# techpro-studio/NNToolkitCore

Hardware: AMD Instinct MI355X
Metric: audio frames/sec (whole node) (higher is better)
Workload: dtype f32

## Files before the change

### nntoolkitcore_amd/csrc/hip/conv1d_kernels.hpp

```cpp
#pragma once
#include "nntk_common.hpp"
#include <stdlib.h>
#include <type_traits>

#define CONV_BM 128
#define CONV_KC 16
#define CONV_LS (CONV_KC + 4)

struct ConvParams {
    const float *in;
    long in_seq, in_row;
    const float *wp;
    const float *bias;
    const float *bn;
    float *out;
    float bn_eps;
    float relu_a;
    int act_kind;
    int B, T, Cin, Cin_p, Cout, Cout_p, k, stride, Tout;
    int tiles_per_seq;
    int m_tiles, n_tiles;
    int out_mode;
    int rows_a;
    int bn_fast;
// ... 276 lines not shown
    if (fast_store) {
        if (!p.bn && p.act_kind == NNTK_ACT_IDENTITY) epilogue(F_{}, AId{}, T_{});
        else if (p.bn && p.act_kind == NNTK_ACT_RELU) epilogue(T_{}, ARelu{}, T_{});
        else if (p.bn)                                epilogue(T_{}, AAny{}, T_{});
        else                                          epilogue(F_{}, AAny{}, T_{});
    } else {
        if (p.bn) epilogue(T_{}, AAny{}, F_{});
        else      epilogue(F_{}, AAny{}, F_{});
    }
}

typedef __bf16 cf3_bf16x2 __attribute__((ext_vector_type(2)));
typedef float cf3_f32x2 __attribute__((ext_vector_type(2)));
__device__ __forceinline__ unsigned cf3_cvt_pk(float a, float b) {
    return __builtin_bit_cast(unsigned, __builtin_convertvector((cf3_f32x2){a, b}, cf3_bf16x2));
}
__device__ __forceinline__ void cf3_split_pair(float x0, float x1, unsigned &hi, unsigned &mid, unsigned &lo) {
#pragma clang fp contract(off)
    hi = cf3_cvt_pk(x0, x1);
    const float r0 = x0 - __uint_as_float(hi << 16), r1 = x1 - __uint_as_float(hi & 0xffff0000u);
    mid = cf3_cvt_pk(r0, r1);
    const float s0 = r0 - __uint_as_float(mid << 16), s1 = r1 - __uint_as_float(mid & 0xffff0000u);
    lo = cf3_cvt_pk(s0, s1);
}

#define CONV_F3_BB 8
#define CONV_F3_TT 16
#ifndef CONV_F3_TMAJOR
#define CONV_F3_BL(m) ((m) & 7)
#define CONV_F3_TL(m) ((m) >> 3)
#else
#define CONV_F3_BL(m) ((m) >> 4)
#define CONV_F3_TL(m) ((m) & 15)
#endif

template <int TM, int TN, int WN>
__device__ __forceinline__ void conv_epilogue_frag3(const ConvParams &p, f32x16 (&acc)[TM][TN], int b0, int x0, int n0,
                                                    int wm, int wn, int l31, int kh, const float *cst) {
    constexpr int BN = WN * TN * 32;
    const size_t total = (size_t)p.Tout * p.f3_nht * p.f3_nks * 3 * 1024;
    const __amdgpu_buffer_rsrc_t rs_out = conv_rsrc(p.out, total);
    auto epilogue = [&](auto bn_tag, auto act_tag) {
        constexpr bool HAS_BN = decltype(bn_tag)::value;
        constexpr int ACT = decltype(act_tag)::value;
        int row_voff[TM];
#pragma unroll
        for (int i = 0; i < TM; ++i) {
            const int m = (wm * TM + i) * 32 + l31;
            const int b = b0 + CONV_F3_BL(m), x = x0 + CONV_F3_TL(m);
            row_voff[i] = (b < p.B && x < p.Tout) ? (int)((((size_t)x * p.f3_nht + (b >> 5)) * p.f3_nks * 3) * 1024) + (32 * kh + (b & 31)) * 16
                                                  : CONV_OOB;
        }
#pragma unroll
        for (int j = 0; j < TN; ++j) {
#pragma unroll
            for (int gp = 0; gp < 2; ++gp) {
                const int cu = n0 + (wn * TN + j) * 32 + 16 * gp;
                const bool ks_ok = cu < p.Cout;
                const int ks_off = (cu >> 4) * 3 * 1024;
                unsigned img[TM][2][3][2];
#pragma unroll
                for (int s = 0; s < 2; ++s) {
                    const int g = 2 * gp + s;
                    const int cb = cu + 8 * s + 4 * kh;
                    const int cl = (wn * TN + j) * 32 + 8 * g + 4 * kh;
                    const float4 bias4 = *reinterpret_cast<const float4 *>(cst + cl);
                    const float bias[4] = {bias4.x, bias4.y, bias4.z, bias4.w};
                    float ga[4] = {1.f, 1.f, 1.f, 1.f}, be[4] = {0.f, 0.f, 0.f, 0.f}, mu[4] = {0.f, 0.f, 0.f, 0.f},
                          sd[4] = {1.f, 1.f, 1.f, 1.f}, rsd[4] = {1.f, 1.f, 1.f, 1.f};
                    if (HAS_BN) {
                        const float4 t1 = *reinterpret_cast<const float4 *>(cst + BN + cl);
                        const float4 t2 = *reinterpret_cast<const float4 *>(cst + 2 * BN + cl);
                        const float4 t3 = *reinterpret_cast<const float4 *>(cst + 3 * BN + cl);
                        const float4 t4 = *reinterpret_cast<const float4 *>(cst + 4 * BN + cl);
                        const float4 t5 = *reinterpret_cast<const float4 *>(cst + 5 * BN + cl);
                        ga[0] = t1.x; ga[1] = t1.y; ga[2] = t1.z; ga[3] = t1.w;
                        be[0] = t2.x; be[1] = t2.y; be[2] = t2.z; be[3] = t2.w;
                        mu[0] = t3.x; mu[1] = t3.y; mu[2] = t3.z; mu[3] = t3.w;
                        sd[0] = t4.x; sd[1] = t4.y; sd[2] = t4.z; sd[3] = t4.w;
                        rsd[0] = t5.x; rsd[1] = t5.y; rsd[2] = t5.z; rsd[3] = t5.w;
                    }
#pragma unroll
                    for (int i = 0; i < TM; ++i) {
                        float v[4];
#pragma unroll
                        for (int e = 0; e < 4; ++e) {
                            v[e] = acc[i][j][4 * g + e] + bias[e];
                            if (HAS_BN) {
                                const float d = v[e] - mu[e];
                                float qn = d * rsd[e];
                                qn = fmaf(fmaf(-qn, sd[e], d), rsd[e], qn);
                                v[e] = p.bn_fast ? (d * rsd[e]) * ga[e] + be[e] : nofma_muladd(qn, ga[e], be[e]);
                            }
                            v[e] = ACT == -1 ? nntk_act(p.act_kind, v[e], p.relu_a)
                                 : ACT == NNTK_ACT_RELU ? nntk_act(NNTK_ACT_RELU, v[e], p.relu_a)
                                 : v[e];
                            if (cb + e >= p.Cout) v[e] = 0.0f;
                        }
                        cf3_split_pair(v[0], v[1], img[i][s][0][0], img[i][s][1][0], img[i][s][2][0]);
                        cf3_split_pair(v[2], v[3], img[i][s][0][1], img[i][s][1][1], img[i][s][2][1]);
                    }
                }
#pragma unroll
                for (int i = 0; i < TM; ++i) {
#pragma unroll
                    for (int im = 0; im < 3; ++im) {
                        const auto s01 = __builtin_amdgcn_permlane32_swap(img[i][0][im][0], img[i][1][im][0], false, false);
                        const auto s23 = __builtin_amdgcn_permlane32_swap(img[i][0][im][1], img[i][1][im][1], false, false);
                        const v4u32_t pk = {s01[0], s23[0], s01[1], s23[1]};
                        const int vo = (ks_ok && row_voff[i] != CONV_OOB) ? row_voff[i] + ks_off + im * 1024 : CONV_OOB;
                        __builtin_amdgcn_raw_buffer_store_b128(pk, rs_out, vo, 0, 0);
                    }
                }
            }
        }
    };
    using T_ = std::true_type; using F_ = std::false_type;
    using AId = std::integral_constant<int, NNTK_ACT_IDENTITY>;
    using ARelu = std::integral_constant<int, NNTK_ACT_RELU>;
    using AAny = std::integral_constant<int, -1>;
    if (!p.bn && p.act_kind == NNTK_ACT_IDENTITY) epilogue(F_{}, AId{});
    else if (p.bn && p.act_kind == NNTK_ACT_RELU) epilogue(T_{}, ARelu{});
    else if (p.bn)                                epilogue(T_{}, AAny{});
    else                                          epilogue(F_{}, AAny{});
}

template <int WM, int WN, int TM, int TN, bool A4, bool QUAD, int AMAX = 192>
__global__ __launch_bounds__(256, 2) void conv1d_mfma_kernel(ConvParams p) {
    constexpr int BN = WN * TN * 32;
    constexpr int KC = CONV_KC, LS = CONV_LS;
    static_assert(WM * WN == 4, "4 wavefronts per workgroup");
    static_assert(WM * TM * 32 == CONV_BM, "BM = 128");
    extern __shared__ __attribute__((aligned(16))) float smem[];
    const int a_elems = p.rows_a * LS;
    constexpr int w_elems = BN * LS;
    const int w_base = 2 * a_elems;

    const int tid = threadIdx.x;
    const int lane = tid & 63;
    const int wave = __builtin_amdgcn_readfirstlane(tid >> 6);
    const int wm = wave / WN, wn = wave % WN;
    const int l31 = lane & 31, kh = lane >> 5;

    const int xcd = blockIdx.x & 7, local = blockIdx.x >> 3;
    const int tile = (local / p.n_tiles) * 8 + xcd;
    if (tile >= p.m_tiles) return;
    const int b = tile / p.tiles_per_seq;
    const int x0 = (tile % p.tiles_per_seq) * CONV_BM;
    const int n0 = (local % p.n_tiles) * BN;
    const int Ktot = p.k * p.Cin_p;


    f32x16 acc[TM][TN];

    constexpr int A_TPR = A4 ? KC / 4 : KC;
    constexpr int AR_STEP = 256 / A_TPR;
    constexpr int A_PT = (AMAX + AR_STEP - 1) / AR_STEP;
    constexpr int W_PT = (BN * (KC / 4) + 255) / 256;
    constexpr bool W_ALL = (BN * (KC / 4)) % 256 == 0;
    const int ac = A4 ? (tid % A_TPR) * 4 : (tid % A_TPR);
    const int ar = tid / A_TPR;
    const int wr = tid >> 2, wc4 = tid & 3;
    v4u32_t areg4[A4 ? A_PT : 1];
    unsigned areg[A4 ? 1 : A_PT];
    v4u32_t wreg[W_PT];
    int a_voff[A_PT], w_voff[W_PT];
#pragma unroll
    for (int q = 0; q < A_PT; ++q) a_voff[q] = (int)(((long)(ar + q * AR_STEP) * p.in_row + ac) * 4);
#pragma unroll
    for (int q = 0; q < W_PT; ++q) w_voff[q] = ((wr + q * 64) * Ktot + wc4 * 4) * 4;
    const bool cin_ragged = (p.Cin % KC) != 0;

    const int n_cchunks = p.Cin_p / KC;
    const int n_chunks = n_cchunks * p.k;
    const int last_blocks = (((p.Cin + 7) & ~7) - (n_cchunks - 1) * KC + 7) / 8;

    const __amdgpu_buffer_rsrc_t rs_w = conv_rsrc(p.wp, (size_t)p.Cout_p * Ktot * 4);
    auto load_w = [&](int tn0, int cc, int kk) {
        const int soff = (tn0 * Ktot + kk * p.Cin_p + cc * KC) * 4;
#pragma unroll
        for (int q = 0; q < W_PT; ++q)
            if (W_ALL || tid + q * 256 < BN * (KC / 4))
                wreg[q] = __builtin_amdgcn_raw_buffer_load_b128(rs_w, w_voff[q], soff, 0);
    };
    const size_t in_total = (size_t)p.B * p.T * p.Cin;
    auto load_a = [&](int tb, int tx0, int cc) {
        const size_t in_off = (size_t)tb * p.in_seq + (size_t)tx0 * p.stride * p.in_row;
        const __amdgpu_buffer_rsrc_t rs_in = conv_rsrc(p.in + in_off, (in_total - in_off) * 4);
        const int soff = cc * KC * 4;
        if (cin_ragged && cc == n_cchunks - 1) {
            const bool ch_ok = cc * KC + ac < p.Cin;
#pragma unroll
            for (int q = 0; q < A_PT; ++q) {
                const int vo = ch_ok ? a_voff[q] : CONV_OOB;
                if (A4) areg4[q] = __builtin_amdgcn_raw_buffer_load_b128(rs_in, vo, soff, 0);
                else    areg[q] = __builtin_amdgcn_raw_buffer_load_b32(rs_in, vo, soff, 0);
            }
        } else {
#pragma unroll
            for (int q = 0; q < A_PT; ++q) {
                if (A4) areg4[q] = __builtin_amdgcn_raw_buffer_load_b128(rs_in, a_voff[q], soff, 0);
                else    areg[q] = __builtin_amdgcn_raw_buffer_load_b32(rs_in, a_voff[q], soff, 0);
            }
        }
    };

    const int a_rd = ((wm * TM * 32 + l31) * p.stride) * LS + 4 * kh;
    const int w_rd = w_base + (wn * TN * 32 + l31) * LS + 4 * kh;
    const int a_tile = 32 * p.stride * LS;

    load_a(b, x0, 0);
    load_w(n0, 0, 0);
    float *cst = smem + 2 * a_elems + 2 * w_elems;
    {
        float c[6];
        conv_load_constants<BN>(p, n0, tid, c);
        conv_stage_constants<BN>(cst, tid, c);
    }
#pragma unroll
    for (int i = 0; i < TM; ++i)
#pragma unroll
        for (int j = 0; j < TN; ++j)
#pragma unroll
            for (int r = 0; r < 16; ++r) acc[i][j][r] = 0.0f;
    int cc = 0, kk = 0;
    for (int chunk = 0; chunk < n_chunks; ++chunk) {
        const int wbuf = chunk & 1;
        const int abuf = cc & 1;
        if (kk == 0) {
            float *As = smem + abuf * a_elems;
#pragma unroll
            for (int q = 0; q < A_PT; ++q) {
                const int r = ar + q * AR_STEP;
                if (r < p.rows_a) {
                    if (A4) *reinterpret_cast<v4u32_t *>(As + r * LS + ac) =
                                (cin_ragged && cc == n_cchunks - 1) ? mask_channels(areg4[q], p.Cin - (cc * KC + ac)) : areg4[q];
                    else    *reinterpret_cast<unsigned *>(As + r * LS + ac) = areg[q];
                }
            }
        }
        {
            float *Ws = smem + w_base + wbuf * w_elems;
#pragma unroll
            for (int q = 0; q < W_PT; ++q)
                if (W_ALL || tid + q * 256 < BN * (KC / 4))
                    *reinterpret_cast<v4u32_t *>(Ws + (wr + q * 64) * LS + wc4 * 4) = wreg[q];
        }
        __syncthreads();
        int ncc = cc, nkk = kk + 1;
        if (nkk == p.k) { nkk = 0; ncc = cc + 1; }
        if (chunk + 1 < n_chunks && !CONV_DBG(4)) {
            load_w(n0, ncc, nkk);
            if (nkk == 0) load_a(b, x0, ncc);
        }
        const float *A = smem + abuf * a_elems + kk * LS + a_rd;
        const float *W = smem + wbuf * w_elems + w_rd;
        auto block8 = [&](int s) {
            float4 a[TM], w[TN];
#pragma unroll
            for (int i = 0; i < TM; ++i) a[i] = *reinterpret_cast<const float4 *>(A + i * a_tile + s);
#pragma unroll
            for (int j = 0; j < TN; ++j) w[j] = *reinterpret_cast<const float4 *>(W + j * 32 * LS + s);
#pragma unroll
            for (int u = 0; u < 4; ++u)
#pragma unroll
                for (int i = 0; i < TM; ++i)
#pragma unroll
                    for (int j = 0; j < TN; ++j) {
                        const float av = u == 0 ? a[i].x : u == 1 ? a[i].y : u == 2 ? a[i].z : a[i].w;
                        const float wv = u == 0 ? w[j].x : u == 1 ? w[j].y : u == 2 ? w[j].z : w[j].w;
                        acc[i][j] = QUAD ? __builtin_amdgcn_mfma_f32_32x32x2f32(wv, av, acc[i][j], 0, 0, 0)
                                         : __builtin_amdgcn_mfma_f32_32x32x2f32(av, wv, acc[i][j], 0, 0, 0);
                    }
        };
        if (!CONV_DBG(2)) {
        block8(0);
        if (cc != n_cchunks - 1 || last_blocks > 1) block8(8);
        }
        cc = ncc; kk = nkk;
    }

    if (CONV_DBG(1) && acc[0][0][0] != 12345.678f) return;
    if constexpr (QUAD) conv_epilogue<TM, TN, WN>(p, acc, b, x0, n0, wm, wn, l31, kh, cst);
    else conv_epilogue_rows<TM, TN, WN>(p, acc, b, x0, n0, wm, wn, l31, kh, cst);
}

typedef __bf16 bf16x8_t __attribute__((ext_vector_type(8)));
typedef __bf16 bf16x2_t __attribute__((ext_vector_type(2)));
typedef float f32x2_t __attribute__((ext_vector_type(2)));

__device__ __forceinline__ unsigned cvt_pk_bf16(float a, float b) {
    return __builtin_bit_cast(unsigned, __builtin_convertvector((f32x2_t){a, b}, bf16x2_t));
}
__device__ __forceinline__ void split3_pair(float x0, float x1, unsigned &hi, unsigned &mid, unsigned &lo) {
    hi = cvt_pk_bf16(x0, x1);
    const float r0 = x0 - __uint_as_float(hi << 16), r1 = x1 - __uint_as_float(hi & 0xffff0000u);
    mid = cvt_pk_bf16(r0, r1);
    const float s0 = r0 - __uint_as_float(mid << 16), s1 = r1 - __uint_as_float(mid & 0xffff0000u);
    lo = cvt_pk_bf16(s0, s1);
}

#define SPLIT_ROW 96

template <int WM, int WN, int TM, int TN, bool A4, bool QUAD, int AMAX = 192, bool F3OUT = false>
__global__ __launch_bounds__(256, 2) void conv1d_mfma_bf16x3_kernel(ConvParams p) {
    constexpr int BN = WN * TN * 32;
    constexpr int KC = CONV_KC;
    static_assert(WM * WN == 4 && WM * TM * 32 == CONV_BM, "4 wavefronts, BM = 128");
    static_assert(!F3OUT || QUAD, "the frag3 epilogue is written for the quad orientation");
    extern __shared__ __attribute__((aligned(16))) float smem[];
    char *lds = reinterpret_cast<char *>(smem);
    const int a_bytes = p.rows_a * SPLIT_ROW;
    constexpr int w_bytes = (BN / 32) * 3 * 1024;
    const int w_base = 2 * a_bytes;

    const int tid = threadIdx.x;
    const int lane = tid & 63;
    const int wave = __builtin_amdgcn_readfirstlane(tid >> 6);
    const int wm = wave / WN, wn = wave % WN;
    const int l31 = lane & 31, kh = lane >> 5;

    const int xcd = blockIdx.x & 7, local = blockIdx.x >> 3;
#ifndef CONV_F3_INTERLEAVED
    const int tile = F3OUT ? xcd * ((p.m_tiles + 7) >> 3) + local / p.n_tiles : (local / p.n_tiles) * 8 + xcd;
#else
    const int tile = (local / p.n_tiles) * 8 + xcd;
#endif
    if (tile >= p.m_tiles) return;
    const int b = F3OUT ? (tile / p.tiles_per_seq) * CONV_F3_BB : tile / p.tiles_per_seq;
    const int x0 = (tile % p.tiles_per_seq) * (F3OUT ? CONV_F3_TT : CONV_BM);
    const int n0 = (local % p.n_tiles) * BN;
    const int Ktot = p.k * p.Cin_p;
    const int ksteps = Ktot >> 4, cin_steps = p.Cin_p >> 4;
    const int wrows = CONV_F3_TT + p.k - 1;

    f32x16 acc[TM][TN];

    constexpr int A_TPR = A4 ? KC / 4 : KC;
    constexpr int AR_STEP = 256 / A_TPR;
    constexpr int A_PT = (AMAX + AR_STEP - 1) / AR_STEP;
    const int ac = A4 ? (tid % A_TPR) * 4 : (tid % A_TPR);
    const int ar = tid / A_TPR;
    v4u32_t areg4[A4 ? A_PT : 1];
    unsigned areg[A4 ? 1 : A_PT];
    constexpr int W_CT = (BN / 32 + 3) / 4;
    v4u32_t wreg[W_CT][3];
    int a_voff[A_PT];
#pragma unroll
    for (int q = 0; q < A_PT; ++q) {
        const int r = ar + q * AR_STEP;
        if (F3OUT) {
            const int bl = r / wrows, tr = r - bl * wrows;
            a_voff[q] = (r < p.rows_a && b + bl < p.B) ? (int)(((long)bl * p.in_seq + (long)tr * p.in_row + ac) * 4) : CONV_OOB;
        } else {
            a_voff[q] = (int)(((long)r * p.in_row + ac) * 4);
        }
    }
    const bool cin_ragged = (p.Cin % KC) != 0;
    const int n_cchunks = p.Cin_p / KC;
    const int n_chunks = n_cchunks * p.k;

    const size_t w_elems_total = (size_t)p.Cout_p * Ktot;
    const int img_bytes = (int)(w_elems_total * 2);
    const __amdgpu_buffer_rsrc_t rs_w = conv_rsrc(p.wp + w_elems_total, (size_t)3 * img_bytes);
    const bool w_thread = wave < BN / 32;
    int w_voff[W_CT];
#pragma unroll
    for (int c = 0; c < W_CT; ++c)
        w_voff[c] = wave + 4 * c < BN / 32 ? (((n0 >> 5) + wave + 4 * c) * ksteps) * 1024 + lane * 16 : CONV_OOB;
    auto load_w = [&](int cc, int kk) {
        const int soff = (kk * cin_steps + cc) * 1024;
#pragma unroll
        for (int c = 0; c < W_CT; ++c)
#pragma unroll
            for (int m = 0; m < 3; ++m) wreg[c][m] = __builtin_amdgcn_raw_buffer_load_b128(rs_w, w_voff[c], soff + m * img_bytes, 0);
    };
    const size_t in_total = (size_t)p.B * p.T * p.Cin;
    const size_t in_off = (size_t)b * p.in_seq + (size_t)x0 * p.stride * p.in_row;
    const __amdgpu_buffer_rsrc_t rs_in = conv_rsrc(p.in + in_off, (in_total - in_off) * 4);
    auto load_a = [&](int cc) {
        const bool ch_ok = !(cin_ragged && cc == n_cchunks - 1) || cc * KC + ac < p.Cin;
#pragma unroll
        for (int q = 0; q < A_PT; ++q) {
            const int vo = ch_ok ? a_voff[q] : CONV_OOB;
            if (A4) areg4[q] = __builtin_amdgcn_raw_buffer_load_b128(rs_in, vo, cc * KC * 4, 0);
            else    areg[q] = __builtin_amdgcn_raw_buffer_load_b32(rs_in, vo, cc * KC * 4, 0);
        }
    };
    auto stage_a = [&](char *As, int nvalid) {
#pragma unroll
        for (int q = 0; q < A_PT; q += (A4 ? 1 : 2)) {
            const int r = ar + q * AR_STEP;
            if (A4) {
                if (r < p.rows_a) {
                    const v4u32_t x = nvalid < 4 ? mask_channels(areg4[q], nvalid) : areg4[q];
                    unsigned h0, m0, l0, h1, m1, l1;
                    split3_pair(__uint_as_float(x.x), __uint_as_float(x.y), h0, m0, l0);
                    split3_pair(__uint_as_float(x.z), __uint_as_float(x.w), h1, m1, l1);
                    char *dst = As + r * SPLIT_ROW + 16 * ((ac >> 3) ^ ((r >> 3) & 1)) + (ac & 7) * 2;
                    *reinterpret_cast<uint2 *>(dst) = make_uint2(h0, h1);
                    *reinterpret_cast<uint2 *>(dst + 32) = make_uint2(m0, m1);
                    *reinterpret_cast<uint2 *>(dst + 64) = make_uint2(l0, l1);
                }
            } else {
                unsigned h, m, l;
                split3_pair(__uint_as_float(areg[q]), __uint_as_float(areg[q + 1 < A_PT ? q + 1 : q]), h, m, l);
#pragma unroll
                for (int e = 0; e < 2; ++e) {
                    const int re = r + e * AR_STEP;
                    if (q + e < A_PT && re < p.rows_a) {
                        char *dst = As + re * SPLIT_ROW + 16 * ((ac >> 3) ^ ((re >> 3) & 1)) + (ac & 7) * 2;
                        *reinterpret_cast<unsigned short *>(dst) = (unsigned short)(e ? h >> 16 : h);
                        *reinterpret_cast<unsigned short *>(dst + 32) = (unsigned short)(e ? m >> 16 : m);
                        *reinterpret_cast<unsigned short *>(dst + 64) = (unsigned short)(e ? l >> 16 : l);
                    }
                }
            }
        }
    };

    const int a_row0 = (wm * TM * 32 + l31) * p.stride;
    int a_row_f3[TM];
#pragma unroll
    for (int i = 0; i < TM; ++i) {
        const int m = (wm * TM + i) * 32 + l31;
        a_row_f3[i] = CONV_F3_BL(m) * wrows + CONV_F3_TL(m);
    }
    const int w_rd = w_base + (wn * TN * 3) * 1024 + lane * 16;
    const int w_wr = w_base + (wave * 3) * 1024 + lane * 16;

    load_a(0);
    load_w(0, 0);
    float *cst = reinterpret_cast<float *>(lds + 2 * a_bytes + 2 * w_bytes);
    {
        float c[6];
        conv_load_constants<BN>(p, n0, tid, c);
        conv_stage_constants<BN>(cst, tid, c);
    }
#pragma unroll
    for (int i = 0; i < TM; ++i)
#pragma unroll
        for (int j = 0; j < TN; ++j)
#pragma unroll
            for (int r = 0; r < 16; ++r) acc[i][j][r] = 0.0f;
    int cc = 0, kk = 0;
    for (int chunk = 0; chunk < n_chunks; ++chunk) {
        const int wbuf = chunk & 1;
        const int abuf = cc & 1;
        if (kk == 0 && !CONV_DBG(16)) stage_a(lds + abuf * a_bytes, (cin_ragged && cc == n_cchunks - 1) ? p.Cin - (cc * KC + ac) : 4);
        if (w_thread) {
#pragma unroll
            for (int c = 0; c < W_CT; ++c) {
                char *dst = lds + wbuf * w_bytes + w_wr + c * 4 * 3 * 1024;
#pragma unroll
                for (int m = 0; m < 3; ++m) *reinterpret_cast<v4u32_t *>(dst + 1024 * m) = wreg[c][m];
            }
        }
        __syncthreads();
        int ncc = cc, nkk = kk + 1;
        if (nkk == p.k) { nkk = 0; ncc = cc + 1; }
        if (chunk + 1 < n_chunks) {
            if (!CONV_DBG(4)) load_w(ncc, nkk);
            if (nkk == 0 && !CONV_DBG(32)) load_a(ncc);
        }
        const char *Ab = lds + abuf * a_bytes;
        const char *Wb = lds + wbuf * w_bytes + w_rd;
        bf16x8_t a[3][TM], w[3][TN];
#pragma unroll
        for (int i = 0; i < TM; ++i) {
            const int row = F3OUT ? a_row_f3[i] + kk : a_row0 + i * 32 * p.stride + kk;
            const char *src = Ab + row * SPLIT_ROW + 16 * (kh ^ ((row >> 3) & 1));
#pragma unroll
            for (int m = 0; m < 3; ++m)
                if (!CONV_DBG(8)) a[m][i] = *reinterpret_cast<const bf16x8_t *>(src + 32 * m);
                else a[m][i] = __builtin_bit_cast(bf16x8_t, wreg[0][m]);
        }
#pragma unroll
        for (int j = 0; j < TN; ++j)
#pragma unroll
            for (int m = 0; m < 3; ++m)
                if (!CONV_DBG(8)) w[m][j] = *reinterpret_cast<const bf16x8_t *>(Wb + (j * 3 + m) * 1024);
                else w[m][j] = __builtin_bit_cast(bf16x8_t, wreg[0][m]);
        constexpr int PA[6] = {2, 0, 1, 1, 0, 0};
        constexpr int PW[6] = {0, 2, 1, 0, 1, 0};
        if (!CONV_DBG(2)) {
#pragma unroll
            for (int t = 0; t < 6; ++t)
#pragma unroll
                for (int i = 0; i < TM; ++i)
#pragma unroll
                    for (int j = 0; j < TN; ++j)
                        acc[i][j] = QUAD ? __builtin_amdgcn_mfma_f32_32x32x16_bf16(w[PW[t]][j], a[PA[t]][i], acc[i][j], 0, 0, 0)
                                         : __builtin_amdgcn_mfma_f32_32x32x16_bf16(a[PA[t]][i], w[PW[t]][j], acc[i][j], 0, 0, 0);
        } else {
#pragma unroll
            for (int i = 0; i < TM; ++i)
#pragma unroll
                for (int j = 0; j < TN; ++j)
#pragma unroll
                    for (int m = 0; m < 3; ++m)
                        acc[i][j][m] += __builtin_bit_cast(v4u32_t, a[m][i]).x + __builtin_bit_cast(v4u32_t, w[m][j]).x;
        }
        cc = ncc; kk = nkk;
    }
    if (CONV_DBG(1) && acc[0][0][0] != 12345.678f) return;
    if constexpr (F3OUT) conv_epilogue_frag3<TM, TN, WN>(p, acc, b, x0, n0, wm, wn, l31, kh, cst);
    else if constexpr (QUAD) {
        v4u32_t *epi = nullptr;
#ifndef CONV_EPI_DIRECT
        if (2 * a_bytes + 2 * w_bytes >= CONV_EPI_LDS_BYTES && p.out_mode == 0) {
            __syncthreads();
            epi = reinterpret_cast<v4u32_t *>(lds);
        }
#endif
        conv_epilogue<TM, TN, WN>(p, acc, b, x0, n0, wm, wn, l31, kh, cst, epi);
    }
    else conv_epilogue_rows<TM, TN, WN>(p, acc, b, x0, n0, wm, wn, l31, kh, cst);
}

template <int WM, int WN, int TM, int TN, bool A4>
static int launch_mfma_f3(const ConvParams &p) {
    constexpr int BN = WN * TN * 32;
    size_t lds = (size_t)2 * (p.rows_a * SPLIT_ROW + (BN / 32) * 3 * 1024) + 6 * BN * sizeof(float);
    ConvParams q = p;
    q.m_tiles = ((p.B + CONV_F3_BB - 1) / CONV_F3_BB) * p.tiles_per_seq;
    q.n_tiles = p.Cout_p / BN;
    const long blocks = (long)((q.m_tiles + 7) / 8) * 8 * q.n_tiles;
    if ((long)((p.B + CONV_F3_BB - 1) / CONV_F3_BB) * p.tiles_per_seq > 0x7fffffffL / 8 || blocks > 0x7fffffffL)
        return nntk_fail_msg("conv1d: too many tiles for one launch");
    auto kern = conv1d_mfma_bf16x3_kernel<WM, WN, TM, TN, A4, true, 192, true>;
    if (lds > 64 * 1024) {
        if (nntk_set_max_dynamic_lds((const void *)kern, lds)) return -1;
    }
    hipLaunchKernelGGL(kern, dim3((unsigned)blocks), dim3(256), lds, nntk_stream(), q);
    NNTK_LAUNCH_CHECK("conv1d_mfma_bf16x3_kernel<frag3>");
    nntk_set_last_conv_kernel("conv1d_mfma_bf16x3_kernel<frag3>");
    return 0;
}

template <int WM, int WN, int TM, int TN, bool A4, bool SPLIT, bool QUAD, int AMAX = 192>
static int launch_mfma_o(const ConvParams &p) {
    constexpr int BN = WN * TN * 32;
    size_t lds = SPLIT ? (size_t)2 * (p.rows_a * SPLIT_ROW + (BN / 32) * 3 * 1024)
                       : (size_t)(2 * p.rows_a * CONV_LS + 2 * BN * CONV_LS) * sizeof(float);
    lds += 6 * BN * sizeof(float);
    ConvParams q = p;
    q.m_tiles = p.B * p.tiles_per_seq;
    q.n_tiles = p.Cout_p / BN;
    const long blocks = (long)((q.m_tiles + 7) / 8) * 8 * q.n_tiles;
    if ((long)p.B * p.tiles_per_seq > 0x7fffffffL / 8 || blocks > 0x7fffffffL)
        return nntk_fail_msg("conv1d: too many tiles for one launch");
    auto kern = SPLIT ? conv1d_mfma_bf16x3_kernel<WM, WN, TM, TN, A4, QUAD, AMAX> : conv1d_mfma_kernel<WM, WN, TM, TN, A4, QUAD, AMAX>;
    if (lds > 64 * 1024) {
        if (nntk_set_max_dynamic_lds((const void *)kern, lds)) return -1;
    }
    dim3 grid((unsigned)blocks);
    hipLaunchKernelGGL(kern, grid, dim3(256), lds, nntk_stream(), q);
    NNTK_LAUNCH_CHECK("conv1d_mfma_kernel");
    nntk_set_last_conv_kernel(SPLIT ? "conv1d_mfma_bf16x3_kernel" : "conv1d_mfma_kernel");
    return 0;
}


int nntk_conv1d_launch_s2(const ConvParams &p, bool a4, bool split);
```

### nntoolkitcore_amd/csrc/hip/nntk_common.hpp

```cpp
#pragma once
#include <hip/hip_runtime.h>
#include <math.h>
#include "nntk_shim.h"

hipStream_t nntk_stream();
int nntk_fail(const char *what, hipError_t err);
int nntk_fail_msg(const char *what);
enum { NNTK_SPAN_REC = 0, NNTK_SPAN_SPEC = 1 };
int nntk_prof_span_begin(int kind);
void nntk_prof_span_end(int idx, long launches, long units);

struct NntkOptions {
    int rec_persistent = -1;
    int rec_xw = -1;
    int rec_pingpong = -1;
    int rec_groups = 2;
    int rec_spin_us = 1000000;
    int rec_stream = -1;
    int rec_fused2 = -1;
    int rec_rr = -1;
    int rec_xf = -1;
    int rec_fk = -1;
    int rec_hf = -1;
    int rec_hf_pend = 1;
    int rec_bd = -1;
    int dense_frag3 = -1;
    int dense_f16x2 = -1;
    int train_outer_plain = -1;
    int train_bptt = -1;
    int spec_ppw = 0;
    int spec_variant = -1;
#ifdef NNTK_VARIANT_SPEC_DMA
    int spec_dma = -1;
#endif
    int bn_fast = 0;
    int gemm_tm_batch = -1;
    int conv_a4 = 1;
    int conv_flatk = -1;
    int conv_frag3_out = -1;
    int conv_store = -1;
    int gemm_split_bf16 = -1;
    int gemm_wide = -1;
    int conv_dbg = 0;
    int weights_check = -1;
};
const NntkOptions &nntk_options();

unsigned *nntk_fault_word();
int nntk_fault_enqueue_copy();
int nntk_persistent_disabled();
void nntk_persistent_launch_begin();
void nntk_persistent_launch_end();
bool nntk_weights_exact_only(const void *d_wp);
int nntk_cu_count();
void nntk_set_last_conv_kernel(const char *name);
void nntk_set_last_rec_kernel(const char *name);
int nntk_set_max_dynamic_lds(const void *kernel, size_t bytes);
int nntk_outer_mfma_launch(const float *d_A, const float *d_B, float *d_partial, long rows, int I, int K, int a_shift_T,
                           long rps, long seq_pitch, long row_pitch);
int nntk_resident_blocks(const void *kernel, int threads, size_t lds, int max_per_cu);

#define NNTK_STR_(x) #x
#define NNTK_STR(x) NNTK_STR_(x)

#define NNTK_HIP_TRY(expr)                                             \
    do {                                                               \
        hipError_t _e = (expr);                                        \
        if (_e != hipSuccess) return nntk_fail(#expr, _e);             \
    } while (0)

#define NNTK_LAUNCH_CHECK(name)                                        \
    do {                                                               \
        hipError_t _e = hipGetLastError();                             \
        if (_e != hipSuccess) return nntk_fail(name, _e);              \
    } while (0)

typedef float f32x4 __attribute__((ext_vector_type(4)));
typedef float f32x16 __attribute__((ext_vector_type(16)));

__device__ __forceinline__ float nntk_act(int kind, float x, float relu_a) {
    switch (kind) {
    case NNTK_ACT_SIGMOID: return 1.0f / (1.0f + expf(-x));
    case NNTK_ACT_TANH:    return tanhf(x);
    case NNTK_ACT_RELU: {
        float y = fmaxf(x, 0.0f);
        return relu_a != 1.0f ? y * relu_a : y;
    }
    case NNTK_ACT_LOG_EPS: return logf(x + relu_a);
    default: return x;
    }
}

__device__ __forceinline__ float nntk_fast_sigmoid(float x) {
    return __builtin_amdgcn_rcpf(1.0f + __builtin_amdgcn_exp2f(-1.44269504088896341f * x));
}
__device__ __forceinline__ float nntk_fast_tanh(float x) {
    const float e = __builtin_amdgcn_exp2f(-2.88539008177792681f * fabsf(x));
    const float r = (1.0f - e) * __builtin_amdgcn_rcpf(1.0f + e);
    return copysignf(r, x);
}
__device__ __forceinline__ float nntk_gate_act(int kind, float x, float a = 1.0f) {
    switch (kind) {
    case NNTK_ACT_SIGMOID: return nntk_fast_sigmoid(x);
    case NNTK_ACT_TANH:    return nntk_fast_tanh(x);
    case NNTK_ACT_RELU: {
        const float y = fmaxf(x, 0.0f);
        return a != 1.0f ? y * a : y;
    }
    default: return x;
    }
}

static inline int nntk_cdiv(long a, long b) { return (int)((a + b - 1) / b); }
```

### nntoolkitcore_amd/csrc/hip/runtime.hip

```cpp
#include "nntk_common.hpp"
#include <stdio.h>
#include <string.h>
#include <vector>

#include <atomic>
#include <mutex>
#include <stdlib.h>

static thread_local hipStream_t t_stream = nullptr;
static thread_local char g_err[512] = "";

hipStream_t nntk_stream() { return t_stream; }

int nntk_fail(const char *what, hipError_t err) {
    snprintf(g_err, sizeof(g_err), "HIP error in %s: %s", what, hipGetErrorString(err));
    return -1;
}
int nntk_fail_msg(const char *what) {
    snprintf(g_err, sizeof(g_err), "%s", what);
    return -1;
}

static NntkOptions g_opt;
static std::once_flag g_opt_once;
static std::mutex g_opt_mutex;

struct OptDesc { const char *name; const char *env; int NntkOptions::*field; };
static const OptDesc g_opt_table[] = {
    {"rec_persistent", "NNTK_REC_PERSISTENT", &NntkOptions::rec_persistent},
    {"rec_xw", "NNTK_REC_XW", &NntkOptions::rec_xw},
    {"rec_pingpong", "NNTK_REC_PINGPONG", &NntkOptions::rec_pingpong},
    {"rec_groups", "NNTK_REC_GROUPS", &NntkOptions::rec_groups},
    {"rec_spin_us", "NNTK_REC_SPIN_US", &NntkOptions::rec_spin_us},
    {"rec_stream", "NNTK_REC_STREAM", &NntkOptions::rec_stream},
    {"rec_fused2", "NNTK_REC_FUSED2", &NntkOptions::rec_fused2},
    {"rec_rr", "NNTK_REC_RR", &NntkOptions::rec_rr},
    {"rec_xf", "NNTK_REC_XF", &NntkOptions::rec_xf},
    {"rec_fk", "NNTK_REC_FK", &NntkOptions::rec_fk},
    {"rec_hf", "NNTK_REC_HF", &NntkOptions::rec_hf},
    {"rec_hf_pend", "NNTK_REC_HF_PEND", &NntkOptions::rec_hf_pend},
    {"rec_bd", "NNTK_REC_BD", &NntkOptions::rec_bd},
    {"dense_frag3", "NNTK_DENSE_FRAG3", &NntkOptions::dense_frag3},
    {"dense_f16x2", "NNTK_DENSE_F16X2", &NntkOptions::dense_f16x2},
    {"train_bptt", "NNTK_TRAIN_BPTT", &NntkOptions::train_bptt},
    {"train_outer_plain", "NNTK_TRAIN_OUTER_PLAIN", &NntkOptions::train_outer_plain},
    {"spec_ppw", "NNTK_SPEC_PPW", &NntkOptions::spec_ppw},
    {"spec_variant", "NNTK_SPEC_VARIANT", &NntkOptions::spec_variant},
#ifdef NNTK_VARIANT_SPEC_DMA
    {"spec_dma", "NNTK_SPEC_DMA", &NntkOptions::spec_dma},
#endif
    {"bn_fast", "NNTK_BN_FAST", &NntkOptions::bn_fast},
    {"gemm_tm_batch", "NNTK_GEMM_TM_BATCH", &NntkOptions::gemm_tm_batch},
    {"gemm_split_bf16", "NNTK_GEMM_SPLIT_BF16", &NntkOptions::gemm_split_bf16},
    {"conv_store", "NNTK_CONV_STORE", &NntkOptions::conv_store},
    {"conv_frag3_out", "NNTK_CONV_FRAG3_OUT", &NntkOptions::conv_frag3_out},
    {"conv_flatk", "NNTK_CONV_FLATK", &NntkOptions::conv_flatk},
    {"conv_a4", "NNTK_CONV_A4", &NntkOptions::conv_a4},
    {"gemm_wide", "NNTK_GEMM_WIDE", &NntkOptions::gemm_wide},
    {"conv_dbg", "NNTK_CONV_DBG", &NntkOptions::conv_dbg},
    {"weights_check", "NNTK_WEIGHTS_CHECK", &NntkOptions::weights_check},
};
static void opt_init() {
    for (const OptDesc &d : g_opt_table) {
        const char *e = getenv(d.env);
        if (e && *e && strcmp(e, "auto") != 0 && strcmp(e, "default") != 0) g_opt.*(d.field) = atoi(e);
    }
}
const NntkOptions &nntk_options() {
    std::call_once(g_opt_once, opt_init);
    return g_opt;
}

struct ProfSpan { hipEvent_t a, b; long launches, units; int kind; hipStream_t stream; };
static std::vector<ProfSpan> g_spans;
static std::mutex g_span_mutex;
static std::atomic<bool> g_prof{false};

int nntk_prof_span_begin(int kind) {
    if (!g_prof.load(std::memory_order_relaxed)) return -1;
    ProfSpan s;
    s.launches = 0;
    s.units = 0;
    s.kind = kind;
    s.stream = t_stream;
    if (hipEventCreate(&s.a) != hipSuccess || hipEventCreate(&s.b) != hipSuccess) return -1;
    (void)hipEventRecord(s.a, t_stream);
    std::lock_guard<std::mutex> lk(g_span_mutex);
    g_spans.push_back(s);
    return (int)g_spans.size() - 1;
}
void nntk_prof_span_end(int idx, long launches, long units) {
    std::lock_guard<std::mutex> lk(g_span_mutex);
    if (idx < 0 || idx >= (int)g_spans.size()) return;
    (void)hipEventRecord(g_spans[idx].b, g_spans[idx].stream);
    g_spans[idx].launches = launches;
    g_spans[idx].units = units;
}

static thread_local unsigned *t_fault_dev = nullptr;
static thread_local volatile unsigned *t_fault_host = nullptr;
static std::atomic<int> g_persistent_off{0};

unsigned *nntk_fault_word() {
    if (!t_fault_dev) {
        unsigned *d = nullptr, *h = nullptr;
        if (hipMalloc((void **)&d, 256) != hipSuccess) { (void)hipGetLastError(); return nullptr; }
        if (hipHostMalloc((void **)&h, 256, hipHostMallocDefault) != hipSuccess) { (void)hipFree(d); (void)hipGetLastError(); return nullptr; }
        (void)hipMemset(d, 0, 256);
        h[0] = 0;
        t_fault_host = h;
        t_fault_dev = d;
    }
    return t_fault_dev;
}
int nntk_fault_enqueue_copy() {
    if (!t_fault_dev) return 0;
    NNTK_HIP_TRY(hipMemcpyAsync((void *)t_fault_host, t_fault_dev, sizeof(unsigned), hipMemcpyDeviceToHost, t_stream));
    return 0;
}
int nntk_persistent_disabled() { return g_persistent_off.load(std::memory_order_relaxed); }

static unsigned fault_take() {
    if (!t_fault_host || t_fault_host[0] == 0) return 0;
    const unsigned bits = t_fault_host[0];
    (void)hipMemsetAsync(t_fault_dev, 0, sizeof(unsigned), t_stream);
    (void)hipStreamSynchronize(t_stream);
    t_fault_host[0] = 0;
    if (!g_persistent_off.exchange(1))
        fprintf(stderr, "nntoolkitcore_hip: a persistent recurrent launch timed out waiting for its peer workgroups "
                        "(another kernel held the CUs?); switching this process to the per-timestep recurrent kernels\n");
    return bits;
}
static int post_sync() {
    if (fault_take())
        return nntk_fail_msg("persistent recurrent kernel: a workgroup timed out waiting for its peers; results of the "
                             "recurrent calls since the last successful synchronisation are invalid. Later calls use "
                             "the per-timestep kernels.");
    return 0;
}

static std::mutex g_persist_mutex;
static hipStream_t g_persist_last = nullptr;
static bool g_persist_any = false;
static hipEvent_t g_persist_ev = nullptr;
void nntk_persistent_launch_begin() {
    g_persist_mutex.lock();
    if (g_persist_any && g_persist_last != t_stream) {
        if (!g_persist_ev && hipEventCreateWithFlags(&g_persist_ev, hipEventDisableTiming) != hipSuccess) g_persist_ev = nullptr;
        if (g_persist_ev && hipEventRecord(g_persist_ev, g_persist_last) == hipSuccess)
            (void)hipStreamWaitEvent(t_stream, g_persist_ev, 0);
        (void)hipGetLastError();
    }
}
void nntk_persistent_launch_end() {
    g_persist_last = t_stream;
    g_persist_any = true;
    g_persist_mutex.unlock();
}

int nntk_cu_count() {
    static std::atomic<int> cus[64];
    int dev = 0;
    if (hipGetDevice(&dev) != hipSuccess || dev < 0 || dev >= 64) return 0;
    int c = cus[dev].load(std::memory_order_relaxed);
    if (c == 0) {
        (void)hipDeviceGetAttribute(&c, hipDeviceAttributeMultiprocessorCount, dev);
        cus[dev].store(c, std::memory_order_relaxed);
    }
    return c;
}
int nntk_set_max_dynamic_lds(const void *kernel, size_t bytes) {
    struct Seen { const void *k; size_t bytes; int dev; };
    static std::vector<Seen> seen;
    static std::mutex m;
    int dev = 0;
    (void)hipGetDevice(&dev);
    std::lock_guard<std::mutex> lk(m);
    for (const Seen &s : seen)
        if (s.k == kernel && s.dev == dev && s.bytes >= bytes) return 0;
    hipError_t e = hipFuncSetAttribute(kernel, hipFuncAttributeMaxDynamicSharedMemorySize, (int)bytes);
    if (e != hipSuccess) return nntk_fail("hipFuncSetAttribute(MaxDynamicSharedMemorySize)", e);
    seen.push_back({kernel, bytes, dev});
    return 0;
}

int nntk_resident_blocks(const void *kernel, int threads, size_t lds, int max_per_cu) {
    struct Seen { const void *k; size_t lds; int dev, threads, per_cu; };
    static std::vector<Seen> seen;
    static std::mutex m;
    int dev = 0;
    if (hipGetDevice(&dev) != hipSuccess) { (void)hipGetLastError(); return 0; }
    int per_cu = -1;
    {
        std::lock_guard<std::mutex> lk(m);
        for (const Seen &s : seen)
            if (s.k == kernel && s.dev == dev && s.lds == lds && s.threads == threads) { per_cu = s.per_cu; break; }
    }
    if (per_cu < 0) {
        int n = 0;
        if (hipOccupancyMaxActiveBlocksPerMultiprocessor(&n, kernel, threads, lds) != hipSuccess) { (void)hipGetLastError(); n = 0; }
        per_cu = n;
        std::lock_guard<std::mutex> lk(m);
        seen.push_back({kernel, lds, dev, threads, per_cu});
    }
    if (per_cu > max_per_cu) per_cu = max_per_cu;
    return per_cu * nntk_cu_count();
}

static thread_local const char *t_last_rec_kernel = "";
void nntk_set_last_rec_kernel(const char *name) { t_last_rec_kernel = name; }
static thread_local const char *t_last_conv_kernel = "";
void nntk_set_last_conv_kernel(const char *name) { t_last_conv_kernel = name; }

extern "C" {

int nntk_shim_set_option(const char *name, const char *value) {
    if (!name || !value) return nntk_fail_msg("nntk_hip_set_option: NULL name or value");
    (void)nntk_options();
    std::lock_guard<std::mutex> lk(g_opt_mutex);
    for (const OptDesc &d : g_opt_table)
        if (strcmp(d.name, name) == 0) {
            g_opt.*(d.field) = (strcmp(value, "auto") == 0 || strcmp(value, "default") == 0) ? NntkOptions().*(d.field) : atoi(value);
            if (d.field == &NntkOptions::rec_persistent && g_opt.rec_persistent != 0) g_persistent_off.store(0);
            return 0;
        }
    return nntk_fail_msg("nntk_hip_set_option: unknown option");
}
int nntk_shim_get_option(const char *name, int *value) {
    if (!name || !value) return nntk_fail_msg("nntk_hip_get_option: NULL argument");
    const NntkOptions &o = nntk_options();
    for (const OptDesc &d : g_opt_table)
        if (strcmp(d.name, name) == 0) { *value = o.*(d.field); return 0; }
    return nntk_fail_msg("nntk_hip_get_option: unknown option");
}

void nntk_shim_profile_enable(int on) { g_prof.store(on != 0); }
int nntk_shim_profile_get(const char *name, double *total_ms, long *launches, long *units) {
    const int kind = (name && strcmp(name, "spectrogram") == 0) ? NNTK_SPAN_SPEC : NNTK_SPAN_REC;
    *total_ms = 0.0;
    *launches = 0;
    *units = 0;
    std::lock_guard<std::mutex> lk(g_span_mutex);
    std::vector<ProfSpan> keep;
    for (auto &s : g_spans) {
        if (s.kind != kind) { keep.push_back(s); continue; }
        float ms = 0.f;
        if (hipEventSynchronize(s.b) == hipSuccess && hipEventElapsedTime(&ms, s.a, s.b) == hipSuccess) {
            *total_ms += ms;
            *launches += s.launches;
            *units += s.units;
        }
        (void)hipEventDestroy(s.a);
        (void)hipEventDestroy(s.b);
    }
    g_spans.swap(keep);
    return 0;
}

const char *nntk_shim_error(void) { return g_err; }
void nntk_shim_set_error(const char *msg) { snprintf(g_err, sizeof(g_err), "%s", msg ? msg : ""); }
void nntk_shim_clear_error(void) { g_err[0] = 0; }

int nntk_shim_device_count(void) {
    int n = 0;
    if (hipGetDeviceCount(&n) != hipSuccess) return 0;
    return n;
}
int nntk_shim_set_device(int device) {
    NNTK_HIP_TRY(hipSetDevice(device));
    return 0;
}
const char *nntk_shim_last_rec_kernel(void) { return t_last_rec_kernel; }
const char *nntk_shim_last_conv_kernel(void) { return t_last_conv_kernel; }
int nntk_shim_get_device(void) {
    int dev = -1;
    if (hipGetDevice(&dev) != hipSuccess) { (void)hipGetLastError(); return -1; }
    return dev;
}
void nntk_shim_set_stream(void *stream) { t_stream = (hipStream_t)stream; }
void *nntk_shim_get_stream(void) { return (void *)t_stream; }
int nntk_shim_synchronize(void) {
    NNTK_HIP_TRY(hipStreamSynchronize(t_stream));
    return post_sync();
}
int nntk_shim_take_fault(void) { return fault_take() ? 1 : 0; }
int nntk_shim_persistent_disabled(void) { return nntk_persistent_disabled(); }
int nntk_shim_device_status(void) { return (t_fault_host && t_fault_host[0]) ? 1 : 0; }

void *nntk_shim_malloc(size_t bytes) {
    void *p = nullptr;
    if (bytes == 0) bytes = 16;
    hipError_t e = hipMalloc(&p, bytes);
    if (e != hipSuccess) { nntk_fail("hipMalloc", e); return nullptr; }
    return p;
}
void nntk_shim_free(void *p) {
    if (!p) return;
    nntk_shim_weights_exact_only(p, 0);
    (void)hipFree(p);
}

void *nntk_shim_host_alloc(size_t bytes) {
    void *p = nullptr;
    if (bytes == 0) bytes = 16;
    hipError_t e = hipHostMalloc(&p, bytes, hipHostMallocDefault);
    if (e != hipSuccess) { nntk_fail("hipHostMalloc", e); return nullptr; }
    memset(p, 0, bytes);
    return p;
}
void nntk_shim_host_free(void *p) { if (p) (void)hipHostFree(p); }

int nntk_shim_upload(void *d_dst, const void *h_src, size_t bytes) {
    if (!bytes) return 0;
    NNTK_HIP_TRY(hipMemcpyAsync(d_dst, h_src, bytes, hipMemcpyHostToDevice, t_stream));
    NNTK_HIP_TRY(hipStreamSynchronize(t_stream));
    return 0;
}
int nntk_shim_download_rows(void *h_dst, const void *d_src, size_t spitch, size_t width, size_t height) {
    if (!width || !height) return 0;
    NNTK_HIP_TRY(hipMemcpy2DAsync(h_dst, width, d_src, spitch, width, height, hipMemcpyDeviceToHost, t_stream));
    NNTK_HIP_TRY(hipStreamSynchronize(t_stream));
    return post_sync();
}
int nntk_shim_copy_rows_d2d(void *d_dst, const void *d_src, size_t spitch, size_t width, size_t height) {
    if (!width || !height) return 0;
    NNTK_HIP_TRY(hipMemcpy2DAsync(d_dst, width, d_src, spitch, width, height, hipMemcpyDeviceToDevice, t_stream));
    return 0;
}
int nntk_shim_upload_async(void *d_dst, const void *h_src, size_t bytes) {
    if (!bytes) return 0;
    NNTK_HIP_TRY(hipMemcpyAsync(d_dst, h_src, bytes, hipMemcpyHostToDevice, t_stream));
    return 0;
}
int nntk_shim_download(void *h_dst, const void *d_src, size_t bytes) {
    if (!bytes) return 0;
    NNTK_HIP_TRY(hipMemcpyAsync(h_dst, d_src, bytes, hipMemcpyDeviceToHost, t_stream));
    NNTK_HIP_TRY(hipStreamSynchronize(t_stream));
    return post_sync();
}
int nntk_shim_download_nocheck(void *h_dst, const void *d_src, size_t bytes) {
    if (bytes) NNTK_HIP_TRY(hipMemcpyAsync(h_dst, d_src, bytes, hipMemcpyDeviceToHost, t_stream));
    NNTK_HIP_TRY(hipStreamSynchronize(t_stream));
    return 0;
}
int nntk_shim_copy_d2d(void *d_dst, const void *d_src, size_t bytes) {
    if (!bytes) return 0;
    NNTK_HIP_TRY(hipMemcpyAsync(d_dst, d_src, bytes, hipMemcpyDeviceToDevice, t_stream));
    return 0;
}
int nntk_shim_memset(void *d_ptr, int value, size_t bytes) {
    if (!bytes) return 0;
    NNTK_HIP_TRY(hipMemsetAsync(d_ptr, value, bytes, t_stream));
    return 0;
}

}

#pragma clang fp contract(off)
__global__ __launch_bounds__(256) void bn_kernel_vec4(const float4 *in, const float *__restrict__ bn,
// ... 339 lines not shown
```

Baseline: 73.99 million.

## Process two K-chunks per barrier in bf16x3 conv1d kernel

Adds a KP=2 variant of the split-bf16 conv1d MFMA kernel that stages weights for two consecutive K chunks into four LDS slots and runs both chunks' MFMAs after a single __syncthreads, halving barrier count. Epilogue constants are kept in registers and staged into LDS after the main loop, reusing the weight region. It is enabled by default (conv_kpair=1) only when LDS use is high enough that occupancy is limited anyway and stride is 1. The cost is more registers for a second weight prefetch buffer and more LDS, which could reduce occupancy.

```diff
diff --git a/nntoolkitcore_amd/csrc/hip/conv1d_kernels.hpp b/nntoolkitcore_amd/csrc/hip/conv1d_kernels.hpp
--- a/nntoolkitcore_amd/csrc/hip/conv1d_kernels.hpp
+++ b/nntoolkitcore_amd/csrc/hip/conv1d_kernels.hpp
@@ -602,12 +602,13 @@
 
 #define SPLIT_ROW 96
 
-template <int WM, int WN, int TM, int TN, bool A4, bool QUAD, int AMAX = 192, bool F3OUT = false>
+template <int WM, int WN, int TM, int TN, bool A4, bool QUAD, int AMAX = 192, bool F3OUT = false, int KP = 1>
 __global__ __launch_bounds__(256, 2) void conv1d_mfma_bf16x3_kernel(ConvParams p) {
     constexpr int BN = WN * TN * 32;
     constexpr int KC = CONV_KC;
     static_assert(WM * WN == 4 && WM * TM * 32 == CONV_BM, "4 wavefronts, BM = 128");
     static_assert(!F3OUT || QUAD, "the frag3 epilogue is written for the quad orientation");
+    static_assert(KP == 1 || KP == 2, "one or two chunks per barrier");
     extern __shared__ __attribute__((aligned(16))) float smem[];
     char *lds = reinterpret_cast<char *>(smem);
     const int a_bytes = p.rows_a * SPLIT_ROW;
@@ -645,6 +646,7 @@
     unsigned areg[A4 ? 1 : A_PT];
     constexpr int W_CT = (BN / 32 + 3) / 4;
     v4u32_t wreg[W_CT][3];
+    v4u32_t wreg2[KP == 2 ? W_CT : 1][3];
     int a_voff[A_PT];
 #pragma unroll
     for (int q = 0; q < A_PT; ++q) {
@@ -668,13 +670,14 @@
 #pragma unroll
     for (int c = 0; c < W_CT; ++c)
         w_voff[c] = wave + 4 * c < BN / 32 ? (((n0 >> 5) + wave + 4 * c) * ksteps) * 1024 + lane * 16 : CONV_OOB;
-    auto load_w = [&](int cc, int kk) {
+    auto load_w_to = [&](v4u32_t (&dst)[W_CT][3], int cc, int kk) {
         const int soff = (kk * cin_steps + cc) * 1024;
 #pragma unroll
         for (int c = 0; c < W_CT; ++c)
 #pragma unroll
-            for (int m = 0; m < 3; ++m) wreg[c][m] = __builtin_amdgcn_raw_buffer_load_b128(rs_w, w_voff[c], soff + m * img_bytes, 0);
+            for (int m = 0; m < 3; ++m) dst[c][m] = __builtin_amdgcn_raw_buffer_load_b128(rs_w, w_voff[c], soff + m * img_bytes, 0);
     };
+    auto load_w = [&](int cc, int kk) { load_w_to(wreg, cc, kk); };
     const size_t in_total = (size_t)p.B * p.T * p.Cin;
     const size_t in_off = (size_t)b * p.in_seq + (size_t)x0 * p.stride * p.in_row;
     const __amdgpu_buffer_rsrc_t rs_in = conv_rsrc(p.in + in_off, (in_total - in_off) * 4);
@@ -731,12 +734,10 @@
 
     load_a(0);
     load_w(0, 0);
-    float *cst = reinterpret_cast<float *>(lds + 2 * a_bytes + 2 * w_bytes);
-    {
-        float c[6];
-        conv_load_constants<BN>(p, n0, tid, c);
-        conv_stage_constants<BN>(cst, tid, c);
-    }
+    float *cst = reinterpret_cast<float *>(lds + (KP == 2 ? w_base : 2 * a_bytes + 2 * w_bytes));
+    float cst_reg[6];
+    conv_load_constants<BN>(p, n0, tid, cst_reg);
+    if constexpr (KP == 1) conv_stage_constants<BN>(cst, tid, cst_reg);
 #pragma unroll
     for (int i = 0; i < TM; ++i)
 #pragma unroll
@@ -744,6 +745,88 @@
 #pragma unroll
             for (int r = 0; r < 16; ++r) acc[i][j][r] = 0.0f;
     int cc = 0, kk = 0;
+    if constexpr (KP == 2) {
+        auto mma_chunk = [&](const char *Ab, const char *Wb, int kk) {
+            bf16x8_t a[3][TM], w[3][TN];
+#pragma unroll
+            for (int i = 0; i < TM; ++i) {
+                const int row = F3OUT ? a_row_f3[i] + kk : a_row0 + i * 32 * p.stride + kk;
+                const char *src = Ab + row * SPLIT_ROW + 16 * (kh ^ ((row >> 3) & 1));
+#pragma unroll
+                for (int m = 0; m < 3; ++m) a[m][i] = *reinterpret_cast<const bf16x8_t *>(src + 32 * m);
+            }
+#pragma unroll
+            for (int j = 0; j < TN; ++j)
+#pragma unroll
+                for (int m = 0; m < 3; ++m) w[m][j] = *reinterpret_cast<const bf16x8_t *>(Wb + (j * 3 + m) * 1024);
+            constexpr int PA[6] = {2, 0, 1, 1, 0, 0};
+            constexpr int PW[6] = {0, 2, 1, 0, 1, 0};
+#pragma unroll
+            for (int t = 0; t < 6; ++t)
+#pragma unroll
+                for (int i = 0; i < TM; ++i)
+#pragma unroll
+                    for (int j = 0; j < TN; ++j)
+                        acc[i][j] = QUAD ? __builtin_amdgcn_mfma_f32_32x32x16_bf16(w[PW[t]][j], a[PA[t]][i], acc[i][j], 0, 0, 0)
+                                         : __builtin_amdgcn_mfma_f32_32x32x16_bf16(a[PA[t]][i], w[PW[t]][j], acc[i][j], 0, 0, 0);
+        };
+        auto stage_cc = [&](int c) {
+            stage_a(lds + (c & 1) * a_bytes, (cin_ragged && c == n_cchunks - 1) ? p.Cin - (c * KC + ac) : 4);
+        };
+        auto put_w = [&](const v4u32_t (&src)[W_CT][3], int slot) {
+            if (w_thread) {
+#pragma unroll
+                for (int c = 0; c < W_CT; ++c) {
+                    char *dst = lds + slot * w_bytes + w_wr + c * 4 * 3 * 1024;
+#pragma unroll
+                    for (int m = 0; m < 3; ++m) *reinterpret_cast<v4u32_t *>(dst + 1024 * m) = src[c][m];
+                }
+            }
+        };
+        auto next_of = [&](int c, int k_, int &nc, int &nk) {
+            nc = c; nk = k_ + 1;
+            if (nk == p.k) { nk = 0; nc = c + 1; }
+        };
+        int c1, k1;
+        next_of(cc, kk, c1, k1);
+        load_w_to(wreg2, c1, k1);
+        const int n_pairs = n_chunks >> 1;
+        auto pair = [&](int i, auto next_tag) {
+            constexpr int NEXT = decltype(next_tag)::value;
+            const int wslot = (i & 1) * 2;
+            if (kk == 0) stage_cc(cc);
+            else if (k1 == 0) stage_cc(c1);
+            put_w(wreg, wslot);
+            put_w(wreg2, wslot + 1);
+            __syncthreads();
+            int c2 = 0, k2 = 0, c3 = 0, k3 = 0;
+            if constexpr (NEXT >= 1) {
+                next_of(c1, k1, c2, k2);
+                load_w_to(wreg, c2, k2);
+                if constexpr (NEXT == 2) {
+                    next_of(c2, k2, c3, k3);
+                    load_w_to(wreg2, c3, k3);
+                    if (k2 == 0 || k3 == 0) load_a(k2 == 0 ? c2 : c3);
+                }
+            }
+            mma_chunk(lds + (cc & 1) * a_bytes, lds + wslot * w_bytes + w_rd, kk);
+            mma_chunk(lds + (c1 & 1) * a_bytes, lds + (wslot + 1) * w_bytes + w_rd, k1);
+            cc = c2; kk = k2; c1 = c3; k1 = k3;
+        };
+        for (int i = 0; i < n_pairs - 1; ++i) pair(i, std::integral_constant<int, 2>{});
+        if (n_chunks & 1) {
+            pair(n_pairs - 1, std::integral_constant<int, 1>{});
+            const int wslot = (n_pairs & 1) * 2;
+            put_w(wreg, wslot);
+            __syncthreads();
+            mma_chunk(lds + (cc & 1) * a_bytes, lds + wslot * w_bytes + w_rd, kk);
+        } else {
+            pair(n_pairs - 1, std::integral_constant<int, 0>{});
+        }
+        __syncthreads();
+        conv_stage_constants<BN>(cst, tid, cst_reg);
+        __syncthreads();
+    } else
     for (int chunk = 0; chunk < n_chunks; ++chunk) {
         const int wbuf = chunk & 1;
         const int abuf = cc & 1;
@@ -818,23 +901,44 @@
     else conv_epilogue_rows<TM, TN, WN>(p, acc, b, x0, n0, wm, wn, l31, kh, cst);
 }
 
+#define CONV_KPAIR_LDS_MAX (80 * 1024)
+template <int BN, int AMAX>
+static int conv_kpair_fits(const ConvParams &p, size_t lds_one, size_t *lds) {
+    if (BN > 128 || AMAX != 192 || p.k < 2 || p.stride != 1) return 0;
+    const size_t need = (size_t)2 * p.rows_a * SPLIT_ROW + (size_t)4 * (BN / 32) * 3 * 1024;
+    if (need > CONV_KPAIR_LDS_MAX) return 0;
+    *lds = need;
+    return 3 * lds_one > 160 * 1024 ? 1 : 2;
+}
+static bool conv_kpair_takes(int fits, int option) { return fits != 0 && (option >= 2 || (option == 1 && fits == 1)); }
+static const char *conv_split_name(bool f3, int fits, bool paired) {
+    const bool dflt = paired == conv_kpair_takes(fits, NntkOptions().conv_kpair);
+    if (f3) return dflt ? "conv1d_mfma_bf16x3_kernel<frag3>" : paired ? "conv1d_mfma_bf16x3_kernel<frag3,kpair>" : "conv1d_mfma_bf16x3_kernel<frag3,kstep1>";
+    return dflt ? "conv1d_mfma_bf16x3_kernel" : paired ? "conv1d_mfma_bf16x3_kernel<kpair>" : "conv1d_mfma_bf16x3_kernel<kstep1>";
+}
+
 template <int WM, int WN, int TM, int TN, bool A4>
 static int launch_mfma_f3(const ConvParams &p) {
     constexpr int BN = WN * TN * 32;
     size_t lds = (size_t)2 * (p.rows_a * SPLIT_ROW + (BN / 32) * 3 * 1024) + 6 * BN * sizeof(float);
+    size_t lds_pair = 0;
+    const int fits = conv_kpair_fits<BN, 192>(p, lds, &lds_pair);
+    const bool paired = conv_kpair_takes(fits, nntk_options().conv_kpair);
+    if (paired) lds = lds_pair;
     ConvParams q = p;
     q.m_tiles = ((p.B + CONV_F3_BB - 1) / CONV_F3_BB) * p.tiles_per_seq;
     q.n_tiles = p.Cout_p / BN;
     const long blocks = (long)((q.m_tiles + 7) / 8) * 8 * q.n_tiles;
     if ((long)((p.B + CONV_F3_BB - 1) / CONV_F3_BB) * p.tiles_per_seq > 0x7fffffffL / 8 || blocks > 0x7fffffffL)
         return nntk_fail_msg("conv1d: too many tiles for one launch");
-    auto kern = conv1d_mfma_bf16x3_kernel<WM, WN, TM, TN, A4, true, 192, true>;
+    auto kern = paired ? conv1d_mfma_bf16x3_kernel<WM, WN, TM, TN, A4, true, 192, true, (BN <= 128 ? 2 : 1)>
+                       : conv1d_mfma_bf16x3_kernel<WM, WN, TM, TN, A4, true, 192, true>;
     if (lds > 64 * 1024) {
         if (nntk_set_max_dynamic_lds((const void *)kern, lds)) return -1;
     }
     hipLaunchKernelGGL(kern, dim3((unsigned)blocks), dim3(256), lds, nntk_stream(), q);
     NNTK_LAUNCH_CHECK("conv1d_mfma_bf16x3_kernel<frag3>");
-    nntk_set_last_conv_kernel("conv1d_mfma_bf16x3_kernel<frag3>");
+    nntk_set_last_conv_kernel(conv_split_name(true, fits, paired));
     return 0;
 }
 
@@ -844,20 +948,26 @@
     size_t lds = SPLIT ? (size_t)2 * (p.rows_a * SPLIT_ROW + (BN / 32) * 3 * 1024)
                        : (size_t)(2 * p.rows_a * CONV_LS + 2 * BN * CONV_LS) * sizeof(float);
     lds += 6 * BN * sizeof(float);
+    size_t lds_pair = 0;
+    const int fits = SPLIT ? conv_kpair_fits<BN, AMAX>(p, lds, &lds_pair) : 0;
+    const bool paired = conv_kpair_takes(fits, nntk_options().conv_kpair);
+    if (paired) lds = lds_pair;
+    constexpr int KP2 = (SPLIT && BN <= 128 && AMAX == 192) ? 2 : 1;
     ConvParams q = p;
     q.m_tiles = p.B * p.tiles_per_seq;
     q.n_tiles = p.Cout_p / BN;
     const long blocks = (long)((q.m_tiles + 7) / 8) * 8 * q.n_tiles;
     if ((long)p.B * p.tiles_per_seq > 0x7fffffffL / 8 || blocks > 0x7fffffffL)
         return nntk_fail_msg("conv1d: too many tiles for one launch");
-    auto kern = SPLIT ? conv1d_mfma_bf16x3_kernel<WM, WN, TM, TN, A4, QUAD, AMAX> : conv1d_mfma_kernel<WM, WN, TM, TN, A4, QUAD, AMAX>;
+    auto kern = paired ? conv1d_mfma_bf16x3_kernel<WM, WN, TM, TN, A4, QUAD, AMAX, false, KP2>
+              : SPLIT  ? conv1d_mfma_bf16x3_kernel<WM, WN, TM, TN, A4, QUAD, AMAX> : conv1d_mfma_kernel<WM, WN, TM, TN, A4, QUAD, AMAX>;
     if (lds > 64 * 1024) {
         if (nntk_set_max_dynamic_lds((const void *)kern, lds)) return -1;
     }
     dim3 grid((unsigned)blocks);
     hipLaunchKernelGGL(kern, grid, dim3(256), lds, nntk_stream(), q);
     NNTK_LAUNCH_CHECK("conv1d_mfma_kernel");
-    nntk_set_last_conv_kernel(SPLIT ? "conv1d_mfma_bf16x3_kernel" : "conv1d_mfma_kernel");
+    nntk_set_last_conv_kernel(SPLIT ? conv_split_name(false, fits, paired) : "conv1d_mfma_kernel");
     return 0;
 }
 
diff --git a/nntoolkitcore_amd/csrc/hip/nntk_common.hpp b/nntoolkitcore_amd/csrc/hip/nntk_common.hpp
--- a/nntoolkitcore_amd/csrc/hip/nntk_common.hpp
+++ b/nntoolkitcore_amd/csrc/hip/nntk_common.hpp
@@ -37,6 +37,7 @@
     int gemm_tm_batch = -1;
     int conv_a4 = 1;
     int conv_flatk = -1;
+    int conv_kpair = 1;
     int conv_frag3_out = -1;
     int conv_store = -1;
     int gemm_split_bf16 = -1;
diff --git a/nntoolkitcore_amd/csrc/hip/runtime.hip b/nntoolkitcore_amd/csrc/hip/runtime.hip
--- a/nntoolkitcore_amd/csrc/hip/runtime.hip
+++ b/nntoolkitcore_amd/csrc/hip/runtime.hip
@@ -55,6 +55,7 @@
     {"conv_store", "NNTK_CONV_STORE", &NntkOptions::conv_store},
     {"conv_frag3_out", "NNTK_CONV_FRAG3_OUT", &NntkOptions::conv_frag3_out},
     {"conv_flatk", "NNTK_CONV_FLATK", &NntkOptions::conv_flatk},
+    {"conv_kpair", "NNTK_CONV_KPAIR", &NntkOptions::conv_kpair},
     {"conv_a4", "NNTK_CONV_A4", &NntkOptions::conv_a4},
     {"gemm_wide", "NNTK_GEMM_WIDE", &NntkOptions::gemm_wide},
     {"conv_dbg", "NNTK_CONV_DBG", &NntkOptions::conv_dbg},
```

After: 77.85 million, median of 5. 5.2% higher.
